# theovincent/iS-DQN

Measured on AMD Instinct MI355X. Metric: gradient-steps/sec (batch=256, K=9, 84x84x4), higher is better.
Workload: dtype bf16x3 (split-bf16 MFMA operands hi+lo, fp32 accumulate)

## Files before the change

is-dqn_amd/csrc/conv_img.h:

```cpp
#pragma once
#include "net_problems.h"

namespace isdqn {

__device__ __forceinline__ int column_slot(int c16) { return c16 < 4 ? 8 + c16 : (c16 < 12 ? c16 - 4 : c16); }
struct PixelOrder {
    int strips;
    int n_full;
    int full_w;
    FastDiv d_h8, d_rem, d_w;
    PixelOrder() : strips(0), n_full(0), full_w(0) {}
    PixelOrder(int H, int W, bool use_strips) : strips(use_strips ? 1 : 0), n_full(H * 8 * (W / 8)), full_w(8 * (W / 8)) {
        d_h8 = FastDiv((uint32_t)(H * 8));
        d_rem = FastDiv((uint32_t)(W % 8 ? W % 8 : 1));
        d_w = FastDiv((uint32_t)W);
    }
    __device__ __forceinline__ void map(int n, int& y, int& x) const {
        uint32_t a, b;
        if (!strips) {
            d_w.divmod((uint32_t)n, a, b);
            y = (int)a; x = (int)b;
        } else if (n < n_full) {
            d_h8.divmod((uint32_t)n, a, b);
            y = (int)(b >> 3); x = (int)(a * 8 + (b & 7));
        } else {
            d_rem.divmod((uint32_t)(n - n_full), a, b);
            y = (int)a; x = full_w + (int)b;
        }
    }
};

struct ConvImgParams {
    ConvGeom g;
    MatSrc W;
    const float* in;
    FrameSrc fs;
    const float *bias, *gamma, *beta;
    float scale;
    float* act;
    float* z;
    int n_img, z_img;
    int tiles_per_img;
    int R, Wp;
    int PP;
    int plane_elems;
    int ablate;
    FastDiv d_chunk, d_Wp, d_R;
    PixelOrder order;
    long long* stamps;
};

template <int MT, int PASSES, bool U8>
struct ConvImgTraits {
    static constexpr int BM = MT * 16;
    static constexpr int A_PLANES = PASSES >= 2 ? 2 : 1;
    static constexpr int B_PLANES = (PASSES >= 3) ? 2 : 1;
    struct GA {
        static constexpr int PITCH = 48;
        static constexpr int ELEMS = BM * PITCH;
        static constexpr int CHUNKS = BM * (GEMM_BK / 8);
    };
    static constexpr int A_STAGE = A_PLANES * GA::ELEMS;
};

__device__ __forceinline__ void xcd_image_tile(int wg, int n_img, int T, int& j, int& tile) {
    const int full = (n_img / 8) * 8 * T;
    if (T > 1 && wg < full) {
        const int grp = wg / (8 * T), r = wg - grp * 8 * T;
        j = grp * 8 + (r & 7);
        tile = r >> 3;
    } else {
        j = wg / T;
        tile = wg - j * T;
    }
}

template <int NTHR, int PLANES, int BATCH>
__device__ __forceinline__ void fill_image_s8(__bf16* img, int plane_elems, const float* src, int H, int W, int C, int y0, int x0,
                                              int Rl, int Wl, int PP, int tid, const FastDiv& d_cpp, const FastDiv& d_Wl) {
    const int cpp = C >> 3, n_chunks = Rl * Wl * cpp;
    uint32_t pix_u, cc_u, lr_u, xl_u;
    d_cpp.divmod((uint32_t)tid, pix_u, cc_u);
    d_Wl.divmod(pix_u, lr_u, xl_u);
    int cc = (int)cc_u, lr = (int)lr_u, xl = (int)xl_u, pix = (int)pix_u;
    uint32_t dpix_u, dcc_u, dpy_u, dpx_u;
    d_cpp.divmod((uint32_t)NTHR, dpix_u, dcc_u);
    d_Wl.divmod(dpix_u, dpy_u, dpx_u);
    const int dpix = (int)dpix_u, dcc = (int)dcc_u, dpy = (int)dpy_u, dpx = (int)dpx_u;
    for (int c0 = tid; c0 - tid < n_chunks; ) {
        float v[BATCH][8];
        int dst[BATCH];
#pragma unroll
        for (int u = 0; u < BATCH; ++u) {
            const bool on = c0 < n_chunks;
            const int iy = y0 + lr, ix = x0 + xl;
            const bool ok = on && iy >= 0 && iy < H && ix >= 0 && ix < W;
            load8_aligned(ok ? src + ((iy * W + ix) * C + cc * 8) : zero_chunk(), v[u]);
            dst[u] = on ? pix * PP + cc * 8 : -1;
            c0 += NTHR;
            cc += dcc;
            const int carry_c = cc >= cpp ? 1 : 0;
            cc -= carry_c ? cpp : 0;
            pix += dpix + carry_c;
            xl += dpx + carry_c;
            lr += dpy;
            const int carry_x = xl >= Wl ? 1 : 0;
            xl -= carry_x ? Wl : 0;
            lr += carry_x;
        }
#pragma unroll
        for (int u = 0; u < BATCH; ++u) {
            bf16x8 hi, lo;
            if constexpr (PLANES >= 2) {
                s8_unpack(v[u], hi, lo);
                if (dst[u] >= 0) *reinterpret_cast<bf16x8*>(img + plane_elems + dst[u]) = lo;
            } else {
                s8_unpack_hi(v[u], hi);
            }
            if (dst[u] >= 0) *reinterpret_cast<bf16x8*>(img + dst[u]) = hi;
        }
    }
}

template <int N>
struct ImagePrefetch {
    float v[N][8];
    int dst[N];
};
template <int NTHR, int N>
__device__ __forceinline__ void request_image_s8(ImagePrefetch<N>& r, const float* src, int H, int W, int C, int y0, int x0, int Rl, int Wl,
                                                 int PP, int tid, const FastDiv& d_cpp, const FastDiv& d_Wl) {
    const int cpp = C >> 3, n_chunks = Rl * Wl * cpp;
    uint32_t pix_u, cc_u, lr_u, xl_u;
    d_cpp.divmod((uint32_t)tid, pix_u, cc_u);
    d_Wl.divmod(pix_u, lr_u, xl_u);
    int cc = (int)cc_u, lr = (int)lr_u, xl = (int)xl_u, pix = (int)pix_u;
    uint32_t dpix_u, dcc_u, dpy_u, dpx_u;
    d_cpp.divmod((uint32_t)NTHR, dpix_u, dcc_u);
    d_Wl.divmod(dpix_u, dpy_u, dpx_u);
    const int dpix = (int)dpix_u, dcc = (int)dcc_u, dpy = (int)dpy_u, dpx = (int)dpx_u;
    int c0 = tid;
#pragma unroll
    for (int u = 0; u < N; ++u) {
        const bool on = c0 < n_chunks;
        const int iy = y0 + lr, ix = x0 + xl;
        const bool ok = on && iy >= 0 && iy < H && ix >= 0 && ix < W;
        load8_aligned(ok ? src + ((iy * W + ix) * C + cc * 8) : zero_chunk(), r.v[u]);
        r.dst[u] = on ? pix * PP + cc * 8 : -1;
        c0 += NTHR;
        cc += dcc;
        const int carry_c = cc >= cpp ? 1 : 0;
        cc -= carry_c ? cpp : 0;
        pix += dpix + carry_c;
        xl += dpx + carry_c;
        lr += dpy;
        const int carry_x = xl >= Wl ? 1 : 0;
        xl -= carry_x ? Wl : 0;
        lr += carry_x;
    }
}
template <int PLANES, int N>
__device__ __forceinline__ void commit_image_s8(__bf16* img, int plane_elems, const ImagePrefetch<N>& r) {
#pragma unroll
    for (int u = 0; u < N; ++u) {
        bf16x8 hi, lo;
        if constexpr (PLANES >= 2) {
            s8_unpack(r.v[u], hi, lo);
            if (r.dst[u] >= 0) *reinterpret_cast<bf16x8*>(img + plane_elems + r.dst[u]) = lo;
        } else {
            s8_unpack_hi(r.v[u], hi);
        }
        if (r.dst[u] >= 0) *reinterpret_cast<bf16x8*>(img + r.dst[u]) = hi;
    }
}

template <int NTHR, int STACK_MAX = 4>
__device__ __forceinline__ void fill_frames_u8(__bf16* img, const FrameSrc& fs, int j, int row_base, int x0, int R, int Wp, int tid,
                                               const FastDiv& d_cpr) {
    constexpr int PB = 2;
    const int cpr = Wp / 8, per_plane = R * cpr, plane = R * Wp;
    const uint8_t* base[STACK_MAX];
#pragma unroll
    for (int c = 0; c < STACK_MAX; ++c) {
        const int id = c < fs.stack ? fs.frame_id(j, c) : -1;
        base[c] = id >= 0 ? fs.frames + (int64_t)id * fs.stride : nullptr;
    }
    const uint8_t* zeros = reinterpret_cast<const uint8_t*>(zero_chunk());
    for (int pb = 0; pb < per_plane; pb += NTHR * PB) {
        unsigned long long raw[PB][STACK_MAX];
        int sh[PB], dst[PB];
#pragma unroll
        for (int k = 0; k < PB; ++k) {
            const int pos = pb + k * NTHR + tid;
            const bool on = pos < per_plane;
            uint32_t lr, cx;
            d_cpr.divmod((uint32_t)(on ? pos : 0), lr, cx);
            const int iy = row_base + (int)lr, ix0 = (int)cx * 8 + x0;
            const bool ok = on && iy >= 0 && iy < fs.H && ix0 > -8 && ix0 < fs.W;
            const int ixc = min(max(ix0, 0), fs.W - 8);
            const int off = iy * fs.W + ixc;
            sh[k] = ix0 - ixc;
            dst[k] = on ? (int)lr * Wp + (int)cx * 8 : -1;
// ... 1092 lines not shown
```

is-dqn_amd/csrc/conv_u8_pair.h:

```cpp
#pragma once
#include "conv_img.h"

namespace isdqn {

constexpr int U8P_PB = 2;

template <int PASSES, int NSTEPS>
__global__ __launch_bounds__(GEMM_THREADS, 4) void conv_fwd_u8_pair_kernel(const ConvImgParams p) {
    ISDQN_EMPTY_KERNEL_RETURN
    constexpr int MT = 2, NT = 2, MTW = MT, NTHR = GEMM_THREADS, STACK_MAX = 4;
    using T = ConvImgTraits<MT, PASSES, true>;
    using GA = typename T::GA;
    extern __shared__ __attribute__((aligned(16))) char smem_raw[];
    __bf16* smem = reinterpret_cast<__bf16*>(smem_raw);
    __bf16* a_stage = smem;
    __bf16* img = smem + 2 * T::A_STAGE;
    const ConvGeom& g = p.g;
    const int tid = threadIdx.x, lane = tid & 63, wave = tid >> 6, grp = lane >> 4;
#if defined(ISDQN_DEV)
#define U8P_STAMP(i)                                                                                 \
    if (p.stamps != nullptr && threadIdx.x == 0) {                                                  \
        p.stamps[(int64_t)blockIdx.x * 8 + (i)] = (long long)__builtin_amdgcn_s_memtime();           \
        if ((i) == 0) p.stamps[(int64_t)blockIdx.x * 8 + 7] = (long long)__builtin_amdgcn_s_memrealtime(); \
    }
#else
#define U8P_STAMP(i)
#endif
    U8P_STAMP(0);
    const int T2 = p.tiles_per_img >> 1;
    int j, tp;
    xcd_image_tile((int)blockIdx.x, p.n_img, T2, j, tp);

    __shared__ __attribute__((aligned(16))) float s_par[3][64];
    float par_v = 0.f;
    {
        const int which = tid >> 6, ch = tid & 63;
        const float* src = which == 0 ? p.bias : which == 1 ? p.gamma : p.beta;
        const bool ok = tid < 192 && ch < g.cout_p && src != nullptr;
        ISDQN_BOUNDS_CHECK(ok ? src + ch : zero_chunk(), 4, 13);
        par_v = *(const ISDQN_GLOBAL float*)(ok ? src + ch : zero_chunk());
    }
    constexpr int nsteps = NSTEPS;
    const int k_last = g.K - 8;
    constexpr int A_PER = (GA::CHUNKS + NTHR - 1) / NTHR;
    int a_row[A_PER], a_var[A_PER], a_lds[A_PER];
    bool a_on[A_PER];
#pragma unroll
    for (int i = 0; i < A_PER; ++i) {
        int c = tid + i * NTHR;
        a_on[i] = c < GA::CHUNKS;
        if (!a_on[i]) c = 0;
        a_row[i] = stash_row(c);
        a_var[i] = (c & 3) * 8;
        a_lds[i] = a_row[i] * GA::PITCH + (c & 3) * 8;
    }
    constexpr int PF = 4;
    float sa[PF][A_PER][8];
    auto fetch = [&](int slot, int k) {
#pragma unroll
        for (int i = 0; i < A_PER; ++i) p.W.load(a_row[i], k + a_var[i], sa[slot][i]);
    };
    auto stash = [&](int slot, int stage) {
        __bf16* a_hi = a_stage + stage * T::A_STAGE;
        __bf16* a_lo = a_hi + GA::ELEMS;
#pragma unroll
        for (int i = 0; i < A_PER; ++i) {
            if (GA::CHUNKS % NTHR != 0 && !a_on[i]) continue;
            bf16x8 hi, lo;
            if constexpr (PASSES >= 2) {
                s8_unpack(sa[slot][i], hi, lo);
                *reinterpret_cast<bf16x8*>(a_lo + a_lds[i]) = lo;
            } else {
                s8_unpack_hi(sa[slot][i], hi);
            }
            *reinterpret_cast<bf16x8*>(a_hi + a_lds[i]) = hi;
        }
    };
    static_assert(NSTEPS >= PF + 2 && NSTEPS % 2 == 0, "ring of four slices + two staged ones");

    const FrameSrc& fs = p.fs;
    const uint8_t* base[STACK_MAX];
#pragma unroll
    for (int c = 0; c < STACK_MAX; ++c) {
        const int id = c < fs.stack ? fs.frame_id(j, c) : -1;
        base[c] = id >= 0 ? fs.frames + (int64_t)id * fs.stride : nullptr;
    }
    const uint8_t* zeros = reinterpret_cast<const uint8_t*>(zero_chunk());
    const int cpr = p.Wp / 8, per_plane = p.R * cpr, plane = p.R * p.Wp;
    unsigned long long raw[U8P_PB][STACK_MAX];
    auto request = [&](int row_base) {
#pragma unroll
        for (int k = 0; k < U8P_PB; ++k) {
            const int pos = k * NTHR + tid;
            const bool on = pos < per_plane;
            uint32_t lr, cx;
            p.d_chunk.divmod((uint32_t)(on ? pos : 0), lr, cx);
            const int iy = row_base + (int)lr, ix0 = (int)cx * 8 - g.pad;
            const bool ok = on && iy >= 0 && iy < fs.H && ix0 > -8 && ix0 < fs.W;
            const int ixc = min(max(ix0, 0), fs.W - 8);
            const int off = iy * fs.W + ixc;
#pragma unroll
            for (int c = 0; c < STACK_MAX; ++c) raw[k][c] = load_u64_unaligned((ok && base[c] != nullptr) ? base[c] + off : zeros);
        }
    };
    auto commit = [&]() {
#pragma unroll
        for (int k = 0; k < U8P_PB; ++k) {
            const int pos = k * NTHR + tid;
            const bool on = pos < per_plane;
            uint32_t lr, cx;
            p.d_chunk.divmod((uint32_t)(on ? pos : 0), lr, cx);
            const int ix0 = (int)cx * 8 - g.pad;
            const int sh = ix0 - min(max(ix0, 0), fs.W - 8);
            const int dst = (int)lr * p.Wp + (int)cx * 8;
#pragma unroll
            for (int c = 0; c < STACK_MAX; ++c) {
                if (c >= fs.stack) continue;
                float v[8];
                FrameSrc::patch8_cvt(raw[k][c], sh, v);
                bf16x8 hi;
                round8(v, hi);
                if (on) *reinterpret_cast<bf16x8*>(img + c * plane + dst) = hi;
            }
        }
    };
    auto tile_rows = [&](int tile) {
        const int oy_min = (int)g.d_wout.div((uint32_t)(tile * 128));
        return oy_min * g.stride - g.pad;
    };

    struct Frags {
        bf16x8 a_hi[MTW], a_lo[MTW], b_hi[NT];
    };

    auto do_tile = [&](auto it_c) {
        constexpr int it = decltype(it_c)::value;
        const int tile = 2 * tp + it;
        const int p0 = tile * 128;
        const int row_base = tile_rows(tile);
        const int full = (p.n_img / 8) * 8;
        const int old_wg8 = j < full ? (j >> 3) * p.tiles_per_img + tile : (j * p.tiles_per_img + tile) >> 3;
        const int rot = (int)((unsigned)old_wg8 % (unsigned)nsteps);
        auto slice = [&](int s) {
            const int k = s + rot;
            return k >= nsteps ? k - nsteps : k;
        };
#pragma unroll
        for (int d = 0; d < PF; ++d) fetch(d, slice(d) * GEMM_BK);
        if constexpr (it == 0) request(row_base);
        commit();
        U8P_STAMP(it == 0 ? 1 : 4);

        int b_org[NT], out_pix[NT];
#pragma unroll
        for (int nt = 0; nt < NT; ++nt) {
            int pp = p0 + wave * 32 + nt * 16 + (lane & 15);
            const bool in_img = pp < g.npix;
            pp = in_img ? pp : g.npix - 1;
            uint32_t oy_u, ox_u;
            g.d_wout.divmod((uint32_t)pp, oy_u, ox_u);
            const int oy = (int)oy_u, ox = (int)ox_u;
            out_pix[nt] = in_img ? oy * g.wout + ox : -1;
            const int ly0 = oy * g.stride - g.pad - row_base;
            const int lx0 = ox * g.stride;
            b_org[nt] = ly0 * p.Wp + lx0;
        }
        f32x4 acc[MTW][NT];
#pragma unroll
        for (int mt = 0; mt < MTW; ++mt)
#pragma unroll
            for (int nt = 0; nt < NT; ++nt) mfma_init(acc[mt][nt]);

        auto read_frags = [&](int stage, int kk, Frags& f) {
            const __bf16* a_hi = a_stage + stage * T::A_STAGE;
            const __bf16* a_lo = a_hi + GA::ELEMS;
#pragma unroll
            for (int mt = 0; mt < MTW; ++mt) {
                f.a_hi[mt] = read_frag<false, GA::PITCH>(a_hi, mt * 16, lane);
                if constexpr (PASSES >= 2) f.a_lo[mt] = read_frag<false, GA::PITCH>(a_lo, mt * 16, lane);
            }
            int kq = kk * GEMM_BK + grp * 8;
            kq = kq < k_last ? kq : k_last;
            const int c = kq >> 6, ky = (kq >> 3) & 7;
            const int tap_off = (c * p.R + ky) * p.Wp;
#pragma unroll
            for (int nt = 0; nt < NT; ++nt) {
                const __bf16* src = img + b_org[nt] + tap_off;
                typedef __attribute__((ext_vector_type(4))) __bf16 bf16x4;
                bf16x4 h0 = *reinterpret_cast<const bf16x4*>(src);
                bf16x4 h1 = *reinterpret_cast<const bf16x4*>(src + 4);
                f.b_hi[nt] = __builtin_shufflevector(h0, h1, 0, 1, 2, 3, 4, 5, 6, 7);
            }
        };
        auto mfma_step = [&](const Frags& f) {
#pragma unroll
            for (int nt = 0; nt < NT; ++nt)
#pragma unroll
                for (int mt = 0; mt < MTW; ++mt) {
                    if constexpr (PASSES >= 2) mfma_acc(acc[mt][nt], f.a_lo[mt], f.b_hi[nt]);
                    mfma_acc(acc[mt][nt], f.a_hi[mt], f.b_hi[nt]);
                }
        };
        Frags fr[2];
        if constexpr (it == 0) {
            if (tid < 192) s_par[tid >> 6][tid & 63] = par_v;
        }
        stash(0, 0);
        stash(1, 1);
        fetch(0, slice(PF) * GEMM_BK);
        fetch(1, slice(PF + 1) * GEMM_BK);
        __syncthreads();
        read_frags(0, slice(0), fr[0]);
        __syncthreads();
#pragma unroll
        for (int s = 0; s < NSTEPS; ++s) {
            if (s + 1 < NSTEPS) read_frags((s + 1) & 1, slice(s + 1), fr[(s + 1) & 1]);
            mfma_step(fr[s & 1]);
            if (s + 2 < NSTEPS) stash((s + 2) % PF, s & 1);
            if (s + 2 + PF < NSTEPS) fetch((s + 2) % PF, slice(s + 2 + PF) * GEMM_BK);
            if constexpr (it == 0) {
                if (s == NSTEPS - 3) request(tile_rows(tile + 1));
            }
            constexpr int N_MFMA = MTW * NT * (PASSES >= 3 ? 3 : PASSES);
#pragma unroll
            for (int i = 0; i < N_MFMA; ++i) {
                __builtin_amdgcn_sched_group_barrier(0x008, 1, 0);
                if (i < N_MFMA / 2) __builtin_amdgcn_sched_group_barrier(0x100, 1, 0);
                __builtin_amdgcn_sched_group_barrier(0x002, 2, 0);
            }
            __syncthreads();
        }

        U8P_STAMP(it == 0 ? 2 : 5);
        float bi[MTW][4], ga[MTW][4], be[MTW][4];
#pragma unroll
        for (int mt = 0; mt < MTW; ++mt) {
            const int ch0 = (mt * 16 + grp * 4) & 63;
            const float4 b4 = *reinterpret_cast<const float4*>(&s_par[0][ch0]);
            const float4 g4 = *reinterpret_cast<const float4*>(&s_par[1][ch0]);
            const float4 e4 = *reinterpret_cast<const float4*>(&s_par[2][ch0]);
            bi[mt][0] = b4.x; bi[mt][1] = b4.y; bi[mt][2] = b4.z; bi[mt][3] = b4.w;
            ga[mt][0] = g4.x; ga[mt][1] = g4.y; ga[mt][2] = g4.z; ga[mt][3] = g4.w;
            be[mt][0] = e4.x; be[mt][1] = e4.y; be[mt][2] = e4.z; be[mt][3] = e4.w;
        }
        const float inv_c = 1.0f / (float)g.cout;
        float zv[NT][MTW][4], s1[NT], s2[NT];
#pragma unroll
        for (int nt = 0; nt < NT; ++nt) {
            s1[nt] = s2[nt] = 0.f;
#pragma unroll
            for (int mt = 0; mt < MTW; ++mt)
#pragma unroll
                for (int r = 0; r < 4; ++r) {
                    int ch = mt * 16 + grp * 4 + r;
                    float zz = ch < g.cout ? acc[mt][nt][r] * p.scale + bi[mt][r] : 0.f;
                    zv[nt][mt][r] = zz;
                    s1[nt] += zz;
                    s2[nt] += zz * zz;
                }
            if (p.gamma != nullptr) {
                s1[nt] += __shfl_xor(s1[nt], 16); s1[nt] += __shfl_xor(s1[nt], 32);
                s2[nt] += __shfl_xor(s2[nt], 16); s2[nt] += __shfl_xor(s2[nt], 32);
            }
        }
#pragma unroll
        for (int nt = 0; nt < NT; ++nt) {
            float mean = 0.f, rstd = 1.f;
            if (p.gamma != nullptr) {
                mean = s1[nt] * inv_c;
                float var = fmaxf(s2[nt] * inv_c - mean * mean, 0.f);
                rstd = rsqrtf(var + 1e-6f);
            }
            if (out_pix[nt] >= 0) {
                const int64_t pix = (int64_t)j * g.npix + out_pix[nt];
#pragma unroll
                for (int mt = 0; mt < MTW; ++mt) {
                    int ch0 = mt * 16 + grp * 4;
                    if (ch0 >= g.cout_p) continue;
                    float4 a, zq;
                    float* ap = &a.x;
                    float* zp = &zq.x;
#pragma unroll
                    for (int r = 0; r < 4; ++r) {
                        float y = p.gamma != nullptr ? (zv[nt][mt][r] - mean) * (rstd * ga[mt][r]) + be[mt][r] : zv[nt][mt][r];
                        ap[r] = (ch0 + r < g.cout) ? fmaxf(y, 0.f) : 0.f;
                        zp[r] = zv[nt][mt][r];
                    }
                    s8_store_quad_paired(p.act + pix * g.cout_p, ch0, a.x, a.y, a.z, a.w);
                    if (j < p.z_img) *reinterpret_cast<float4*>(p.z + pix * g.cout_p + ch0) = zq;
                }
            }
        }
        U8P_STAMP(it == 0 ? 3 : 6);
    };
    do_tile(std::integral_constant<int, 0>{});
    do_tile(std::integral_constant<int, 1>{});
#undef U8P_STAMP
}

template <int PASSES, int NSTEPS>
static int launch_conv_fwd_u8_pair(const ConvImgParams& p, hipStream_t st) {
    using T = ConvImgTraits<2, PASSES, true>;
    const int lds = (2 * T::A_STAGE + T::B_PLANES * p.plane_elems) * 2;
    static LdsConfigured configured;
    if (int rc = ensure_dynamic_lds(&conv_fwd_u8_pair_kernel<PASSES, NSTEPS>, lds, configured)) return rc;
    const int grid = p.n_img * (p.tiles_per_img / 2);
    ISDQN_REPORT_OCCUPANCY((&conv_fwd_u8_pair_kernel<PASSES, NSTEPS>), GEMM_THREADS, lds, grid);
    hipLaunchKernelGGL((conv_fwd_u8_pair_kernel<PASSES, NSTEPS>), dim3(grid), dim3(GEMM_THREADS), lds, st, p);
    ISDQN_HIP_CHECK(hipGetLastError());
    return ISDQN_OK;
}

}
```

is-dqn_amd/csrc/net_launch.h:

```cpp
#pragma once
#if defined(ISDQN_DEV)
static long long* g_stamps = nullptr;
static int g_stamp_layer = -1;
static char g_stamp_name[32] = "";
extern "C" int isdqn_debug_set_stamps(void* buf, const char* layer_name) {
    g_stamps = (long long*)buf;
    g_stamp_layer = buf ? 0 : -1;
    snprintf(g_stamp_name, sizeof(g_stamp_name), "%s", layer_name ? layer_name : "");
    return ISDQN_OK;
}
static long long* stamps_for(const char* kernel_tag) {
    return (g_stamp_layer >= 0 && strcmp(kernel_tag, g_stamp_name) == 0) ? g_stamps : nullptr;
}
#else
static long long* stamps_for(const char*) { return nullptr; }
#endif

__global__ __launch_bounds__(256) void split_params_kernel(const float* __restrict__ p, float* __restrict__ mirror, int64_t n_groups) {
    const int64_t g = (int64_t)blockIdx.x * 256 + threadIdx.x;
    if (g >= n_groups) return;
    float v[8];
    load8_aligned(p + g * 8, v);
    s8_store_group(mirror + g * 8, v);
}
static int refresh_mirror(const Plan& P, const float* params, float* ws, hipStream_t st) {
    const int64_t n_groups = P.n_params / 8;
    hipLaunchKernelGGL(split_params_kernel, dim3((unsigned)((n_groups + 255) / 256)), dim3(256), 0, st, params, ws + P.wsplit_off, n_groups);
    ISDQN_HIP_CHECK(hipGetLastError());
    return ISDQN_OK;
}

static ConvGeom conv_geom(const Layer& l) {
    ConvGeom g;
    g.hin = l.hin; g.win = l.win; g.cin_p = l.cin_p; g.hout = l.hout; g.wout = l.wout;
    g.cout = l.cout; g.cout_p = l.cout_p; g.ksz = l.ksz; g.stride = l.stride; g.pad = l.pad;
    g.npix = l.npix; g.K = l.K;
    g.stride_sh = l.stride == 4 ? 2 : l.stride == 2 ? 1 : 0;
    g.d_npix = FastDiv(l.npix); g.d_wout = FastDiv(l.wout); g.d_cinp = FastDiv(l.cin_p);
    g.d_ksz = FastDiv(l.ksz); g.d_coutp = FastDiv(l.cout_p);
    return g;
}

constexpr int DZ_S8 = 1;

struct NetInput {
    const uint8_t* frames; int64_t frame_stride; const int* frame_ids; int paired_B;
    const float* obs; const float* obs2; int obs_split;
    int id_pitch = 0, id_off = 0;
};

template <int BM, int PASSES, bool U8>
static int launch_conv_fwd(const Layer& l, const float* params, const float* wmir, const NetInput& in, const float* act_in, int n_img,
                           int z_img, float* act, float* z, hipStream_t st) {
    ConvFwd<BM, PASSES, U8> p;
    p.g = conv_geom(l);
    p.W = MatSrc{wmir + l.w_off, l.K, l.cout_p, l.K, 1};
    p.in = act_in;
    p.fs = FrameSrc{in.frames, in.frame_stride, in.frame_ids, l.cin, in.paired_B, l.hin, l.win, in.id_pitch, in.id_off};
    p.bias = params + l.b_off;
    p.gamma = l.has_ln ? params + l.g_off : nullptr;
    p.beta = l.has_ln ? params + l.be_off : nullptr;
    p.scale = U8 ? (1.0f / 255.0f) : 1.0f;
    p.act = act; p.z = z;
    p.n_pix_total = n_img * l.npix;
    p.z_pix = z_img * l.npix;
    return launch_gemm(p, ceil_div(p.n_pix_total, 128), st);
}

static int conv_fwd_img(const Layer& l, bool x3, const float* params, const float* wmir, const NetInput& in, const float* act_in, int n_img,
                        int z_img, float* act, float* z, hipStream_t st, bool* done) {
    *done = false;
    if (act == nullptr || (z == nullptr && z_img > 0)) return ISDQN_OK;
    ConvImgParams ip;
    ip.g = conv_geom(l);
    const int mt = l.cout_p <= 32 ? 2 : 4;
    const int passes = x3 ? (l.is_u8 ? 2 : 3) : 1;
    ip.PP = l.is_u8 ? 0 : l.cin_p + (l.cin_p % 64 == 0 ? 16 : 8);
    int lds = conv_img_geometry(ip.g, l.is_u8, l.cin, passes >= 3 ? 2 : 1, mt, passes >= 2 ? 2 : 1, ip.R, ip.Wp,
                                ip.plane_elems, ip.PP);
    constexpr int LDS_LIMIT = 158 * 1024;
    if (lds > LDS_LIMIT || (l.is_u8 && (l.win < 8 || l.cin > 4))) return ISDQN_OK;
    if (!l.is_u8 && l.cin_p < 16) return ISDQN_OK;
    if (!l.is_u8 && l.npix <= 128) {
        const int want = ip.Wp + (((l.wout - ip.Wp) % 8) + 8) % 8;
        const int planes = passes >= 3 ? 2 : 1;
        const int lds2 = lds + planes * ip.R * (want - ip.Wp) * ip.PP * 2;
        const int stage2 = (passes >= 2 ? 2 : 1) * (mt * 16) * 48 * 2 * 2;
        const int old_total = lds > 80 * 1024 ? lds + stage2 : lds, new_total = lds2 > 80 * 1024 ? lds2 + stage2 : lds2;
        if (want != ip.Wp && new_total <= LDS_LIMIT && (old_total <= 80 * 1024) == (new_total <= 80 * 1024)) {
            ip.Wp = want;
            ip.plane_elems = ip.R * want * ip.PP;
            lds = lds2;
        }
    }
    ip.W = MatSrc{wmir + l.w_off, l.K, l.cout_p, l.K, 1};
    ip.in = act_in;
    ip.fs = FrameSrc{in.frames, in.frame_stride, in.frame_ids, l.cin, in.paired_B, l.hin, l.win, in.id_pitch, in.id_off};
    ip.bias = params + l.b_off;
    ip.gamma = l.has_ln ? params + l.g_off : nullptr;
    ip.beta = l.has_ln ? params + l.be_off : nullptr;
    ip.scale = l.is_u8 ? (1.0f / 255.0f) : 1.0f;
    ip.act = act; ip.z = z; ip.n_img = n_img; ip.z_img = z_img;
    ip.tiles_per_img = ceil_div(l.npix, 128);
    ip.d_chunk = FastDiv((uint32_t)(l.is_u8 ? ip.Wp / 8 : l.cin_p / 8));
    ip.d_Wp = FastDiv((uint32_t)ip.Wp);
    ip.d_R = FastDiv((uint32_t)ip.R);
    ip.order = PixelOrder(l.hout, l.wout, !l.is_u8 && ip.tiles_per_img == 1);
    ip.stamps = stamps_for(l.name);
    ip.ablate = 0;
#if defined(ISDQN_DEV)
    if (const char* e = getenv("ISDQN_ABLATE")) ip.ablate = atoi(e);
#endif
    *done = true;
    if (l.is_u8) {
#if !defined(ISDQN_NO_U8_PAIR)
        if (mt == 2 && ip.tiles_per_img % 2 == 0 && ip.R * (ip.Wp / 8) <= U8P_PB * GEMM_THREADS && l.cin == 4 && l.K == 256 && ip.ablate == 0)
            return passes == 2 ? launch_conv_fwd_u8_pair<2, 8>(ip, st) : launch_conv_fwd_u8_pair<1, 8>(ip, st);
#endif
        if (passes == 2) return mt == 2 ? launch_conv_fwd_img<2, 2, true>(ip, st) : launch_conv_fwd_img<4, 2, true>(ip, st);
        return mt == 2 ? launch_conv_fwd_img<2, 1, true>(ip, st) : launch_conv_fwd_img<4, 1, true>(ip, st);
    }
    const int stage_bytes = (passes >= 2 ? 2 : 1) * (mt * 16) * 48 * 2 * 2;
    static const bool no_kg = ISDQN_DEV_ENV("ISDQN_NO_KGROUPS");
    const bool kg2 = !no_kg && mt == 4 && lds > 80 * 1024 && lds + stage_bytes <= LDS_LIMIT &&
                     mt * 16 * 128 * 4 <= lds - stage_bytes && l.K >= 8 * GEMM_BK;
#if !defined(ISDQN_NO_U8_PAIR)
    if (passes == 3 && mt == 4 && kg2 && ip.tiles_per_img == 1 && l.K == 512 && n_img % 2 == 0 && ip.ablate == 0 && ip.stamps == nullptr &&
        ip.R * ip.Wp * (l.cin_p / 8) <= S8P_BATCH * GEMM_THREADS * 2)
        return launch_conv_fwd_s8_pair<8>(ip, st);
#endif
    if (passes == 3) return mt == 2 ? launch_conv_fwd_img<2, 3, false>(ip, st)
                          : kg2 ? launch_conv_fwd_img<4, 3, false, 2>(ip, st) : launch_conv_fwd_img<4, 3, false>(ip, st);
    return mt == 2 ? launch_conv_fwd_img<2, 1, false>(ip, st)
         : kg2 ? launch_conv_fwd_img<4, 1, false, 2>(ip, st) : launch_conv_fwd_img<4, 1, false>(ip, st);
}

static int conv_fwd(const Layer& l, bool x3, const float* params, const float* wmir, const NetInput& in, const float* act_in, int n_img,
                    int z_img, float* act, float* z, hipStream_t st) {
    bool done = false;
    int rc = conv_fwd_img(l, x3, params, wmir, in, act_in, n_img, z_img, act, z, st, &done);
    if (rc || done) return rc;
    const bool small = l.cout_p <= 32;
    if (l.is_u8) {
        if (x3) return small ? launch_conv_fwd<32, 2, true>(l, params, wmir, in, act_in, n_img, z_img, act, z, st)
                             : launch_conv_fwd<64, 2, true>(l, params, wmir, in, act_in, n_img, z_img, act, z, st);
        return small ? launch_conv_fwd<32, 1, true>(l, params, wmir, in, act_in, n_img, z_img, act, z, st)
                     : launch_conv_fwd<64, 1, true>(l, params, wmir, in, act_in, n_img, z_img, act, z, st);
    }
    if (x3) return small ? launch_conv_fwd<32, 3, false>(l, params, wmir, in, act_in, n_img, z_img, act, z, st)
                         : launch_conv_fwd<64, 3, false>(l, params, wmir, in, act_in, n_img, z_img, act, z, st);
    return small ? launch_conv_fwd<32, 1, false>(l, params, wmir, in, act_in, n_img, z_img, act, z, st)
                 : launch_conv_fwd<64, 1, false>(l, params, wmir, in, act_in, n_img, z_img, act, z, st);
}

static int effective_splits(int K, int splits, int* steps_per_split = nullptr) {
    int ksteps = ceil_div(K, GEMM_BK);
    if (splits < 1) splits = 1;
    if (splits > ksteps) splits = ksteps;
    int sps = ceil_div(ksteps, splits);
    if (steps_per_split) *steps_per_split = sps;
    return ceil_div(ksteps, sps);
}

template <int BM, int BN, int WM, int WN, bool ATR, bool BTR, int PASSES, bool AL, bool A2PART, bool ADAM = false, int S8M = 0>
static int launch_plain(const MatSrc& A, const float* A2, int a_split, const MatSrc& B, float* C, int ldc, int M,
                        int N, int K, int splits, int64_t slab_stride, hipStream_t st,
                        const AdamFuse* adam = nullptr) {
    PlainGemm<BM, BN, WM, WN, ATR, BTR, PASSES, AL, A2PART, ADAM, S8M> p;
    if (adam) p.adam = *adam;
    p.A = A; p.B = B; p.A2 = A2; p.a_split = a_split; p.C = C; p.ldc = ldc; p.M = M; p.N = N; p.K = K;
    p.tiles_m = ceil_div(M, BM); p.tiles_n = ceil_div(N, BN);
    p.splits = effective_splits(K, splits, &p.steps_per_split);
    p.slab_stride = slab_stride;
    return launch_gemm(p, p.tiles_m * p.tiles_n * p.splits, st);
}

template <bool ATR, bool BTR, bool AL = true, bool A2PART = false, int S8M = 0>
static int plain_big(bool x3, const MatSrc& A, const float* A2, int a_split, const MatSrc& B, float* C, int ldc,
                     int M, int N, int K, int splits, int64_t slab_stride, hipStream_t st) {
    if (x3)
        return launch_plain<128, 128, 2, 2, ATR, BTR, 3, AL, A2PART, false, S8M>(A, A2, a_split, B, C, ldc, M, N, K, splits,
                                                                                 slab_stride, st);
    return launch_plain<128, 128, 2, 2, ATR, BTR, 1, AL, A2PART, false, S8M>(A, A2, a_split, B, C, ldc, M, N, K, splits,
                                                                             slab_stride, st);
}

template <bool ATR, bool BTR, int S8M = 0>
static int plain_narrow(bool x3, const MatSrc& A, const MatSrc& B, float* C, int ldc, int M, int N, int K, int splits,
                        int64_t slab_stride, hipStream_t st) {
    if (x3) return launch_plain<128, 64, 2, 2, ATR, BTR, 3, true, false, false, S8M>(A, nullptr, 0, B, C, ldc, M, N, K, splits, slab_stride, st);
    return launch_plain<128, 64, 2, 2, ATR, BTR, 1, true, false, false, S8M>(A, nullptr, 0, B, C, ldc, M, N, K, splits, slab_stride, st);
}

static int dense_fwd(const Layer& l, bool x3, const float* params, const float* wmir, const NetInput& in, const float* act_in, int rows,
                     int z_rows, float* slab, float* act, float* z, hipStream_t st, bool skip_post = false) {
    MatSrc A, B;
    const float* A2 = nullptr;
    int a_split = 0;
    if (l.in_unpadded_ld) {
        A = MatSrc{in.obs, l.in_unpadded_ld, rows, l.in_f, 0};
        if (in.obs2) { A2 = in.obs2; a_split = in.obs_split; }
    } else {
        A = MatSrc{act_in, l.in_p, rows, l.in_p, 1};
    }
    B = MatSrc{wmir + l.w_off, l.in_p, l.out_f, l.in_p, 1};
    const int ns = effective_splits(l.in_unpadded_ld ? l.in_f : l.K, l.fwd_splits);
    const int64_t slab_stride = l.out_p;
    const int ldc = ns * l.out_p;
    int rc;
    if (l.in_unpadded_ld) {
        rc = A2 ? plain_big<false, false, false, true, 2>(x3, A, A2, a_split, B, slab, ldc, rows, l.out_f, l.in_f,
                                                          l.fwd_splits, slab_stride, st)
                : plain_big<false, false, false, false, 2>(x3, A, nullptr, 0, B, slab, ldc, rows, l.out_f, l.in_f,
                                                           l.fwd_splits, slab_stride, st);
    } else if (l.fwd_narrow) {
        rc = plain_narrow<false, false, 3>(x3, A, B, slab, ldc, rows, l.out_f, l.K, l.fwd_splits, slab_stride, st);
    } else {
        rc = plain_big<false, false, true, false, 3>(x3, A, nullptr, 0, B, slab, ldc, rows, l.out_f, l.K, l.fwd_splits, slab_stride,
                                                     st);
    }
    if (rc || skip_post) return rc;
    hipLaunchKernelGGL(dense_post_kernel, dim3(rows), dim3(256), 3 * l.out_p * sizeof(float), st, slab, ns, slab_stride,
                       (int64_t)ldc, rows, l.out_f, l.out_p, params + l.b_off, l.has_ln ? params + l.g_off : nullptr,
                       l.has_ln ? params + l.be_off : nullptr, l.has_relu, act, z, z_rows, l.is_head ? 0 : 1);
    ISDQN_HIP_CHECK(hipGetLastError());
    return ISDQN_OK;
}

static int impala_forward(const Plan& P, bool x3, const float* params, const float* wmir, const NetInput& in, int n_img, int z_img,
                          float* ws, hipStream_t st, int bn_mode = 0);
static int bn_forward(const Plan& P, bool x3, const float* params, const NetInput& in, int n_img, int z_img, float* ws, float* q_out, bool running,
                      hipStream_t st);

static float* duel_raw_rows(const Plan& P, float* ws, const float* q_out) {
    const int64_t o = q_out - ws;
    if (o >= P.out_off && o < P.out_off + (int64_t)P.N2 * P.nlog_p) return ws + P.raw_off + (o - P.out_off) / P.nlog_p * P.raw_p;
    if (P.out_t_off >= 0 && o >= P.out_t_off && o < P.out_t_off + (int64_t)P.qt_rows * P.nlog_p)
        return ws + P.raw_t_off + (o - P.out_t_off) / P.nlog_p * P.raw_p;
    return nullptr;
}
static int duel_combine(const Plan& P, const float* raw, float* out, int n_rows, hipStream_t st) {
    const int64_t threads = (int64_t)n_rows * P.n_heads * (P.head_nb > 0 ? P.head_nb : 1);
    hipLaunchKernelGGL(duel_combine_kernel, dim3((unsigned)((threads + DUEL_THREADS - 1) / DUEL_THREADS)), dim3(DUEL_THREADS), 0, st, raw, P.raw_p, out,
                       P.nlog_p, n_rows, P.n_heads, P.n_actions, P.head_nb > 0 ? P.head_nb : 1);
    ISDQN_HIP_CHECK(hipGetLastError());
    return ISDQN_OK;
}

static int net_forward(const Plan& P, bool x3, const float* params, const NetInput& in, int n_img, int z_img,
                       float* ws, float* q_out, hipStream_t st, int n_run = -1, int skip_post_layer = -1) {
    if (P.bn) {
        ISDQN_REQUIRE(n_run < 0 && skip_post_layer < 0, ISDQN_ERR_UNSUPPORTED, "partial forward passes are not built for BatchNorm networks");
        return bn_forward(P, x3, params, in, n_img, z_img, ws, q_out, true, st);
    }
    const float* prev = nullptr;
    const float* wmir = ws + P.wsplit_off;
    if (n_run < 0) n_run = P.n_layers;
    for (int i = 0; i < n_run; ++i) {
        const Layer& l = P.L[i];
        float* act = l.is_head ? q_out : ws + l.act_off;
        float* z = l.is_head ? nullptr : ws + l.z_off;
        int rc;
        if (l.is_head && P.dueling) {
            act = duel_raw_rows(P, ws, q_out);
            ISDQN_REQUIRE(act != nullptr, ISDQN_ERR_ARG, "dueling heads: the head output must go to the workspace's head rows");
        }
        if (l.kind == 2)
            rc = impala_forward(P, x3, params, wmir, in, n_img, z_img, ws, st);
        else if (l.kind == 0)
// ... 439 lines not shown
```

Baseline: 4280.

## Make u8 pair conv keep weights resident in LDS with one block per image

```diff
diff --git a/is-dqn_amd/csrc/conv_img.h b/is-dqn_amd/csrc/conv_img.h
--- a/is-dqn_amd/csrc/conv_img.h
+++ b/is-dqn_amd/csrc/conv_img.h
@@ -48,6 +48,7 @@
     FastDiv d_chunk, d_Wp, d_R;
     PixelOrder order;
     long long* stamps;
+    int Rd;
 };
 
 template <int MT, int PASSES, bool U8>
diff --git a/is-dqn_amd/csrc/conv_u8_pair.h b/is-dqn_amd/csrc/conv_u8_pair.h
--- a/is-dqn_amd/csrc/conv_u8_pair.h
+++ b/is-dqn_amd/csrc/conv_u8_pair.h
@@ -4,19 +4,30 @@
 namespace isdqn {
 
 constexpr int U8P_PB = 2;
+constexpr int U8P_THREADS = 512;
+constexpr int U8P_WPITCH = 256 + 16;
+constexpr int U8P_WPLANE = 32 * U8P_WPITCH;
+
+__host__ __device__ __forceinline__ int u8p_rotation(int j, int tile, int n_img, int tiles_per_img, int nsteps) {
+    const int full = (n_img / 8) * 8;
+    const int old_wg8 = j < full ? (j >> 3) * tiles_per_img + tile : (j * tiles_per_img + tile) >> 3;
+    return (int)((unsigned)old_wg8 % (unsigned)nsteps);
+}
 
 template <int PASSES, int NSTEPS>
-__global__ __launch_bounds__(GEMM_THREADS, 4) void conv_fwd_u8_pair_kernel(const ConvImgParams p) {
+__global__ __launch_bounds__(U8P_THREADS, 4) void conv_fwd_u8_pair_kernel(const ConvImgParams p) {
     ISDQN_EMPTY_KERNEL_RETURN
-    constexpr int MT = 2, NT = 2, MTW = MT, NTHR = GEMM_THREADS, STACK_MAX = 4;
-    using T = ConvImgTraits<MT, PASSES, true>;
-    using GA = typename T::GA;
+    constexpr int MT = 2, NT = 2, MTW = MT, NTHR = U8P_THREADS, STACK_MAX = 4;
+    constexpr int W_PLANES = PASSES >= 2 ? 2 : 1;
+    static_assert(NSTEPS * GEMM_BK == 256, "resident weights: [32][256 k]");
     extern __shared__ __attribute__((aligned(16))) char smem_raw[];
     __bf16* smem = reinterpret_cast<__bf16*>(smem_raw);
-    __bf16* a_stage = smem;
-    __bf16* img = smem + 2 * T::A_STAGE;
+    __bf16* w_hi = smem;
+    __bf16* w_lo = smem + U8P_WPLANE;
+    __bf16* img = smem + W_PLANES * U8P_WPLANE;
     const ConvGeom& g = p.g;
-    const int tid = threadIdx.x, lane = tid & 63, wave = tid >> 6, grp = lane >> 4;
+    const int tid = threadIdx.x, lane = tid & 63, grp = lane >> 4;
+    const int wave = (tid >> 6) & 3, hw = tid >> 8;
 #if defined(ISDQN_DEV)
 #define U8P_STAMP(i)                                                                                 \
     if (p.stamps != nullptr && threadIdx.x == 0) {                                                  \
@@ -27,9 +38,8 @@
 #define U8P_STAMP(i)
 #endif
     U8P_STAMP(0);
-    const int T2 = p.tiles_per_img >> 1;
-    int j, tp;
-    xcd_image_tile((int)blockIdx.x, p.n_img, T2, j, tp);
+    const int j = (int)blockIdx.x;
+    const int n_half = p.tiles_per_img >> 1;
 
     __shared__ __attribute__((aligned(16))) float s_par[3][64];
     float par_v = 0.f;
@@ -42,41 +52,9 @@
     }
     constexpr int nsteps = NSTEPS;
     const int k_last = g.K - 8;
-    constexpr int A_PER = (GA::CHUNKS + NTHR - 1) / NTHR;
-    int a_row[A_PER], a_var[A_PER], a_lds[A_PER];
-    bool a_on[A_PER];
-#pragma unroll
-    for (int i = 0; i < A_PER; ++i) {
-        int c = tid + i * NTHR;
-        a_on[i] = c < GA::CHUNKS;
-        if (!a_on[i]) c = 0;
-        a_row[i] = stash_row(c);
-        a_var[i] = (c & 3) * 8;
-        a_lds[i] = a_row[i] * GA::PITCH + (c & 3) * 8;
-    }
-    constexpr int PF = 4;
-    float sa[PF][A_PER][8];
-    auto fetch = [&](int slot, int k) {
-#pragma unroll
-        for (int i = 0; i < A_PER; ++i) p.W.load(a_row[i], k + a_var[i], sa[slot][i]);
-    };
-    auto stash = [&](int slot, int stage) {
-        __bf16* a_hi = a_stage + stage * T::A_STAGE;
-        __bf16* a_lo = a_hi + GA::ELEMS;
-#pragma unroll
-        for (int i = 0; i < A_PER; ++i) {
-            if (GA::CHUNKS % NTHR != 0 && !a_on[i]) continue;
-            bf16x8 hi, lo;
-            if constexpr (PASSES >= 2) {
-                s8_unpack(sa[slot][i], hi, lo);
-                *reinterpret_cast<bf16x8*>(a_lo + a_lds[i]) = lo;
-            } else {
-                s8_unpack_hi(sa[slot][i], hi);
-            }
-            *reinterpret_cast<bf16x8*>(a_hi + a_lds[i]) = hi;
-        }
-    };
-    static_assert(NSTEPS >= PF + 2 && NSTEPS % 2 == 0, "ring of four slices + two staged ones");
+    float wv[2][8];
+#pragma unroll
+    for (int i = 0; i < 2; ++i) p.W.load((tid >> 5) + i * 16, (tid & 31) * 8, wv[i]);
 
     const FrameSrc& fs = p.fs;
     const uint8_t* base[STACK_MAX];
@@ -86,9 +64,17 @@
         base[c] = id >= 0 ? fs.frames + (int64_t)id * fs.stride : nullptr;
     }
     const uint8_t* zeros = reinterpret_cast<const uint8_t*>(zero_chunk());
-    const int cpr = p.Wp / 8, per_plane = p.R * cpr, plane = p.R * p.Wp;
-    unsigned long long raw[U8P_PB][STACK_MAX];
-    auto request = [&](int row_base) {
+    const int cpr = p.Wp / 8, plane = p.Rd * p.Wp;
+    auto half_rows = [&](int h, int& row_base) {
+        const int oy_min = (int)g.d_wout.div((uint32_t)(h * 256));
+        const int oy_max = (int)g.d_wout.div((uint32_t)(min(g.npix, h * 256 + 256) - 1));
+        row_base = oy_min * g.stride - g.pad;
+        return ((oy_max - oy_min) * g.stride + g.ksz) * cpr;
+    };
+    typedef unsigned long long RawRows[U8P_PB][STACK_MAX];
+    auto request = [&](RawRows& raw, int h) {
+        int row_base = 0;
+        const int per_plane = h < n_half ? half_rows(h, row_base) : 0;
 #pragma unroll
         for (int k = 0; k < U8P_PB; ++k) {
             const int pos = k * NTHR + tid;
@@ -103,10 +89,13 @@
             for (int c = 0; c < STACK_MAX; ++c) raw[k][c] = load_u64_unaligned((ok && base[c] != nullptr) ? base[c] + off : zeros);
         }
     };
-    auto commit = [&]() {
+    auto commit = [&](const RawRows& raw, int h) {
+        int row_base;
+        const int per_plane = half_rows(h, row_base);
 #pragma unroll
         for (int k = 0; k < U8P_PB; ++k) {
             const int pos = k * NTHR + tid;
+            if (pos - lane >= per_plane) continue;
             const bool on = pos < per_plane;
             uint32_t lr, cx;
             p.d_chunk.divmod((uint32_t)(on ? pos : 0), lr, cx);
@@ -124,32 +113,40 @@
             }
         }
     };
-    auto tile_rows = [&](int tile) {
-        const int oy_min = (int)g.d_wout.div((uint32_t)(tile * 128));
-        return oy_min * g.stride - g.pad;
-    };
+
+    RawRows raw0, raw1;
+    request(raw0, 0);
+    request(raw1, 1);
+#pragma unroll
+    for (int i = 0; i < 2; ++i) {
+        const int at = ((tid >> 5) + i * 16) * U8P_WPITCH + (tid & 31) * 8;
+        bf16x8 hi, lo;
+        if constexpr (PASSES >= 2) {
+            s8_unpack(wv[i], hi, lo);
+            *reinterpret_cast<bf16x8*>(w_lo + at) = lo;
+        } else {
+            s8_unpack_hi(wv[i], hi);
+        }
+        *reinterpret_cast<bf16x8*>(w_hi + at) = hi;
+    }
+    if (tid < 192) s_par[tid >> 6][tid & 63] = par_v;
+    commit(raw0, 0);
 
     struct Frags {
         bf16x8 a_hi[MTW], a_lo[MTW], b_hi[NT];
     };
 
-    auto do_tile = [&](auto it_c) {
-        constexpr int it = decltype(it_c)::value;
-        const int tile = 2 * tp + it;
+    auto do_half = [&](int h) {
+        const int tile = 2 * h + hw;
         const int p0 = tile * 128;
-        const int row_base = tile_rows(tile);
-        const int full = (p.n_img / 8) * 8;
-        const int old_wg8 = j < full ? (j >> 3) * p.tiles_per_img + tile : (j * p.tiles_per_img + tile) >> 3;
-        const int rot = (int)((unsigned)old_wg8 % (unsigned)nsteps);
+        if (p0 + wave * 32 >= g.npix) return;
+        int row_base;
+        half_rows(h, row_base);
+        const int rot = u8p_rotation(j, tile, p.n_img, p.tiles_per_img, nsteps);
         auto slice = [&](int s) {
             const int k = s + rot;
             return k >= nsteps ? k - nsteps : k;
         };
-#pragma unroll
-        for (int d = 0; d < PF; ++d) fetch(d, slice(d) * GEMM_BK);
-        if constexpr (it == 0) request(row_base);
-        commit();
-        U8P_STAMP(it == 0 ? 1 : 4);
 
         int b_org[NT], out_pix[NT];
 #pragma unroll
@@ -171,18 +168,16 @@
 #pragma unroll
             for (int nt = 0; nt < NT; ++nt) mfma_init(acc[mt][nt]);
 
-        auto read_frags = [&](int stage, int kk, Frags& f) {
-            const __bf16* a_hi = a_stage + stage * T::A_STAGE;
-            const __bf16* a_lo = a_hi + GA::ELEMS;
+        auto read_frags = [&](int kk, Frags& f) {
 #pragma unroll
             for (int mt = 0; mt < MTW; ++mt) {
-                f.a_hi[mt] = read_frag<false, GA::PITCH>(a_hi, mt * 16, lane);
-                if constexpr (PASSES >= 2) f.a_lo[mt] = read_frag<false, GA::PITCH>(a_lo, mt * 16, lane);
+                f.a_hi[mt] = read_frag<false, U8P_WPITCH>(w_hi + kk * GEMM_BK, mt * 16, lane);
+                if constexpr (PASSES >= 2) f.a_lo[mt] = read_frag<false, U8P_WPITCH>(w_lo + kk * GEMM_BK, mt * 16, lane);
             }
             int kq = kk * GEMM_BK + grp * 8;
             kq = kq < k_last ? kq : k_last;
             const int c = kq >> 6, ky = (kq >> 3) & 7;
-            const int tap_off = (c * p.R + ky) * p.Wp;
+            const int tap_off = (c * p.Rd + ky) * p.Wp;
 #pragma unroll
             for (int nt = 0; nt < NT; ++nt) {
                 const __bf16* src = img + b_org[nt] + tap_off;
@@ -202,36 +197,20 @@
                 }
         };
         Frags fr[2];
-        if constexpr (it == 0) {
-            if (tid < 192) s_par[tid >> 6][tid & 63] = par_v;
-        }
-        stash(0, 0);
-        stash(1, 1);
-        fetch(0, slice(PF) * GEMM_BK);
-        fetch(1, slice(PF + 1) * GEMM_BK);
-        __syncthreads();
-        read_frags(0, slice(0), fr[0]);
-        __syncthreads();
+        read_frags(slice(0), fr[0]);
 #pragma unroll
         for (int s = 0; s < NSTEPS; ++s) {
-            if (s + 1 < NSTEPS) read_frags((s + 1) & 1, slice(s + 1), fr[(s + 1) & 1]);
+            if (s + 1 < NSTEPS) read_frags(slice(s + 1), fr[(s + 1) & 1]);
             mfma_step(fr[s & 1]);
-            if (s + 2 < NSTEPS) stash((s + 2) % PF, s & 1);
-            if (s + 2 + PF < NSTEPS) fetch((s + 2) % PF, slice(s + 2 + PF) * GEMM_BK);
-            if constexpr (it == 0) {
-                if (s == NSTEPS - 3) request(tile_rows(tile + 1));
-            }
-            constexpr int N_MFMA = MTW * NT * (PASSES >= 3 ? 3 : PASSES);
+            constexpr int N_MFMA = MTW * NT * PASSES;
 #pragma unroll
             for (int i = 0; i < N_MFMA; ++i) {
                 __builtin_amdgcn_sched_group_barrier(0x008, 1, 0);
-                if (i < N_MFMA / 2) __builtin_amdgcn_sched_group_barrier(0x100, 1, 0);
-                __builtin_amdgcn_sched_group_barrier(0x002, 2, 0);
-            }
-            __syncthreads();
-        }
-
-        U8P_STAMP(it == 0 ? 2 : 5);
+                __builtin_amdgcn_sched_group_barrier(0x100, PASSES >= 2 ? 1 : 2, 0);
+            }
+        }
+
+        U8P_STAMP(h == 0 ? 2 : 5);
         float bi[MTW][4], ga[MTW][4], be[MTW][4];
 #pragma unroll
         for (int mt = 0; mt < MTW; ++mt) {
@@ -291,22 +270,41 @@
                 }
             }
         }
-        U8P_STAMP(it == 0 ? 3 : 6);
-    };
-    do_tile(std::integral_constant<int, 0>{});
-    do_tile(std::integral_constant<int, 1>{});
+        U8P_STAMP(h == 0 ? 3 : 6);
+    };
+
+    U8P_STAMP(1);
+    for (int h = 0; h < n_half; ++h) {
+        __syncthreads();
+        do_half(h);
+        if (h + 1 < n_half) {
+            __syncthreads();
+            commit(raw1, h + 1);
+            U8P_STAMP(4);
+            if (h + 2 < n_half) request(raw1, h + 2);
+        }
+    }
 #undef U8P_STAMP
+}
+
+template <int PASSES>
+static inline int conv_u8_pair_lds(int Rd, int Wp) {
+    return ((PASSES >= 2 ? 2 : 1) * U8P_WPLANE + 4 * Rd * Wp) * 2;
+}
+static inline int conv_u8_pair_rows(const ConvGeom& g) {
+    int rows = g.npix <= 256 ? g.hout : ((256 + g.wout - 2) / g.wout + 1);
+    if (rows > g.hout) rows = g.hout;
+    return g.stride * (rows - 1) + g.ksz;
 }
 
 template <int PASSES, int NSTEPS>
 static int launch_conv_fwd_u8_pair(const ConvImgParams& p, hipStream_t st) {
-    using T = ConvImgTraits<2, PASSES, true>;
-    const int lds = (2 * T::A_STAGE + T::B_PLANES * p.plane_elems) * 2;
+    const int lds = conv_u8_pair_lds<PASSES>(p.Rd, p.Wp);
     static LdsConfigured configured;
     if (int rc = ensure_dynamic_lds(&conv_fwd_u8_pair_kernel<PASSES, NSTEPS>, lds, configured)) return rc;
-    const int grid = p.n_img * (p.tiles_per_img / 2);
-    ISDQN_REPORT_OCCUPANCY((&conv_fwd_u8_pair_kernel<PASSES, NSTEPS>), GEMM_THREADS, lds, grid);
-    hipLaunchKernelGGL((conv_fwd_u8_pair_kernel<PASSES, NSTEPS>), dim3(grid), dim3(GEMM_THREADS), lds, st, p);
+    const int grid = p.n_img;
+    ISDQN_REPORT_OCCUPANCY((&conv_fwd_u8_pair_kernel<PASSES, NSTEPS>), U8P_THREADS, lds, grid);
+    hipLaunchKernelGGL((conv_fwd_u8_pair_kernel<PASSES, NSTEPS>), dim3(grid), dim3(U8P_THREADS), lds, st, p);
     ISDQN_HIP_CHECK(hipGetLastError());
     return ISDQN_OK;
 }
diff --git a/is-dqn_amd/csrc/net_launch.h b/is-dqn_amd/csrc/net_launch.h
--- a/is-dqn_amd/csrc/net_launch.h
+++ b/is-dqn_amd/csrc/net_launch.h
@@ -108,13 +108,17 @@
     ip.order = PixelOrder(l.hout, l.wout, !l.is_u8 && ip.tiles_per_img == 1);
     ip.stamps = stamps_for(l.name);
     ip.ablate = 0;
+    ip.Rd = 0;
 #if defined(ISDQN_DEV)
     if (const char* e = getenv("ISDQN_ABLATE")) ip.ablate = atoi(e);
 #endif
     *done = true;
     if (l.is_u8) {
 #if !defined(ISDQN_NO_U8_PAIR)
-        if (mt == 2 && ip.tiles_per_img % 2 == 0 && ip.R * (ip.Wp / 8) <= U8P_PB * GEMM_THREADS && l.cin == 4 && l.K == 256 && ip.ablate == 0)
+        ip.Rd = conv_u8_pair_rows(ip.g);
+        const int lds_pair = passes == 2 ? conv_u8_pair_lds<2>(ip.Rd, ip.Wp) : conv_u8_pair_lds<1>(ip.Rd, ip.Wp);
+        if (mt == 2 && ip.tiles_per_img % 2 == 0 && ip.Rd * (ip.Wp / 8) <= U8P_PB * U8P_THREADS && lds_pair <= LDS_LIMIT && l.cin == 4 &&
+            l.K == 256 && ip.ablate == 0)
             return passes == 2 ? launch_conv_fwd_u8_pair<2, 8>(ip, st) : launch_conv_fwd_u8_pair<1, 8>(ip, st);
 #endif
         if (passes == 2) return mt == 2 ? launch_conv_fwd_img<2, 2, true>(ip, st) : launch_conv_fwd_img<4, 2, true>(ip, st);
```

New measurement: 4373 (median of 6 runs). 1.02x the previous value.
